# arnold117/PrimeKG-RGCN-LinkPrediction

Hardware: NVIDIA B200
Metric: rgcn_fwd_bwd_edges_per_sec (higher is better)
Workload: dtype bf16x3-split / f32-accumulate (operands as bf16 hi + lo planes, three tensor-core products, ~17 mantissa bits; gathers, means, loss in f32)

## Files before the change

primekg-rgcn-linkprediction_b200/csrc/aggregate.cu:

```cuda
#include <stdlib.h>

#include <type_traits>

#include "common.cuh"

namespace rgcn {

enum { MIX_NONE = 0, MIX_SUM = 1, MIX_BASIS = 2 };
#ifndef RGCN_TAILPRED_MAX_VPL
#define RGCN_TAILPRED_MAX_VPL 1
#endif
constexpr int kMaxBasis = 8;

struct AggParams {
  const int32_t* rowptr;
  const int32_t* idx;
  const float* edge_w;
  const int32_t* hub_keys;
  const int32_t* hub_chunk_ptr;
  const int32_t* chunk_table;
  const int32_t* row_order;
  int32_t hub_threshold;
  int32_t skip_hubs;
  int32_t n_hubs;
// ... 20 lines not shown
  int32_t out_mode;
  float* partials;
  const float* dotP;
  int64_t ld_dotP;
  float* gc_partial;
  const int32_t* slot;
  int32_t zero_row;
  const float* mp_mask; int64_t ld_mp_mask; float mp_scale;
  void* mp_hi; void* mp_lo; int64_t ld_mp;
  float* mp_colsum;
  const int64_t* list;
  int64_t n_list;
  int32_t list_slices, list_rsplit;
  int64_t list_walkers;
  int32_t list_by_rows;
  int32_t list_overlap_hubs;
  int32_t stream_rel;
  const uint8_t* row_flag;
  const int32_t* hub_filter;
  int32_t hub_unlisted;
};

template <int G, int VPL, bool W, bool SLOT = false>
__global__ void __launch_bounds__(256) hub_partial_kernel(const AggParams p) {
  pdl_enter();
  constexpr int GROUPS = 256 / G;
  __shared__ float4 red[GROUPS][G * VPL];
  const int chunk = blockIdx.x;
  const int4 t = __ldg(reinterpret_cast<const int4*>(p.chunk_table) + chunk);
  const int key = t.x;
  const int r = key % p.R;
  if (p.hub_filter && __ldg(p.hub_filter + key / p.R) == p.hub_unlisted) return;
  const int seg_beg = __ldg(p.rowptr + key), seg_end = __ldg(p.rowptr + key + 1);
  const int c_beg = seg_beg + (chunk - t.y) * kHubChunk;
  const int c_end = min(c_beg + kHubChunk, seg_end);
  const int nvec = p.d >> 2;
  const int lane = threadIdx.x % G, grp = threadIdx.x / G;
  constexpr int PER = kHubChunk / GROUPS;
  const int g_beg = c_beg + grp * PER, g_end = min(g_beg + PER, c_end);
  float4 acc[VPL];
  int vcol[VPL];
#pragma unroll
  for (int k = 0; k < VPL; ++k) {
    acc[k] = make_float4(0.f, 0.f, 0.f, 0.f);
    const int vi = k * G + lane;
    vcol[k] = vi < nvec ? vi * 4 : 0;
  }
  const float* __restrict__ Fb = p.F + (size_t)r * p.src_rel_stride;
// ... 43 lines not shown
    const float* __restrict__ rp = Fb + (size_t)j * ldf;
#pragma unroll
    for (int k = 0; k < VPL; ++k) {
      const float4 v = ldg4(rp + vcol[k]);
      if (W) fma4(acc[k], wv, v); else add4(acc[k], v);
    }
  }
#pragma unroll
  for (int k = 0; k < VPL; ++k) red[grp][k * G + lane] = acc[k];
  __syncthreads();
  for (int vi = threadIdx.x; vi < nvec; vi += 256) {
    float4 s = red[0][vi];
    for (int g = 1; g < GROUPS; ++g) add4(s, red[g][vi]);
    reinterpret_cast<float4*>(p.partials + (size_t)chunk * p.d)[vi] = s;
  }
}

__device__ __forceinline__ void store_vec_to(void* O, void* O_lo, int64_t ldo, int out_mode, int64_t row, int col,
                                             const float4& v) {
  if (out_mode == 0) {
    *reinterpret_cast<float4*>(reinterpret_cast<float*>(O) + row * ldo + col) = v;
    return;
  }
  __nv_bfloat162 a = __floats2bfloat162_rn(v.x, v.y), b = __floats2bfloat162_rn(v.z, v.w);
  uint2 hi;
  hi.x = *reinterpret_cast<uint32_t*>(&a);
  hi.y = *reinterpret_cast<uint32_t*>(&b);
  *reinterpret_cast<uint2*>(reinterpret_cast<__nv_bfloat16*>(O) + row * ldo + col) = hi;
  if (out_mode == 2) {
    const float hx = __uint_as_float(hi.x << 16), hy = __uint_as_float(hi.x & 0xffff0000u);
    const float hz = __uint_as_float(hi.y << 16), hw = __uint_as_float(hi.y & 0xffff0000u);
    a = __floats2bfloat162_rn(v.x - hx, v.y - hy);
    b = __floats2bfloat162_rn(v.z - hz, v.w - hw);
    uint2 lo;
    lo.x = *reinterpret_cast<uint32_t*>(&a);
    lo.y = *reinterpret_cast<uint32_t*>(&b);
    *reinterpret_cast<uint2*>(reinterpret_cast<__nv_bfloat16*>(O_lo) + row * ldo + col) = lo;
  }
}
__device__ __forceinline__ void store_vec(const AggParams& p, int64_t row, int col, const float4& v) {
  store_vec_to(p.O, p.O_lo, p.ldo, p.out_mode, row, col, v);
}

constexpr int agg_min_blocks(int G, int vpl, int mix, bool w) {
  if (mix == MIX_BASIS || vpl > 2) return 1;
  if (vpl == 2) return (mix == MIX_NONE && !w) ? 5 : 4;
  if (G == 32) return mix == MIX_NONE ? 6 : 5;
  return (mix == MIX_SUM && w) ? 3 : 4;
}

template <int G, int VPL, int MIX, bool W, bool SLOT = false, bool MP = false, bool LIST = false, bool MARK = false>
__global__ void __launch_bounds__(256, LIST ? (VPL > 2 ? 1 : 3) : agg_min_blocks(G, VPL, MIX, W) - (((MP || MARK) && agg_min_blocks(G, VPL, MIX, W) > 1) ? 1 : 0))
aggregate_rows_kernel(const AggParams p) {
  static_assert(!MARK || (SLOT && !MP && MIX == MIX_SUM), "marked sources serve the row-sparse backward walk");
  static_assert(!LIST || (MIX == MIX_NONE && !W && !SLOT && !MP), "the listed-rows walk is the unmixed forward form");
  pdl_enter();
  constexpr int GROUPS = 256 / G;
  constexpr int NB = (MIX == MIX_BASIS) ? kMaxBasis : 1;
  constexpr int U0 = (VPL >= 4) ? 2 : (VPL == 2 ? 4 : 8);
  constexpr int U = U0 < G ? U0 : G;
  constexpr bool TAILPRED = MIX != MIX_BASIS && VPL <= RGCN_TAILPRED_MAX_VPL;
  constexpr bool CHAIN = MIX == MIX_SUM && W;
  extern __shared__ float s_comp[];
  const bool with_gc = MIX == MIX_BASIS && p.dotP != nullptr;
  const bool with_cs = MP && MIX == MIX_SUM && p.mp_colsum != nullptr;
  float* s_gc = s_comp + p.R * p.B;
  if (MIX == MIX_BASIS) {
    for (int t = threadIdx.x; t < p.R * p.B; t += 256) s_comp[t] = p.comp[(t / p.B) * p.ldcomp + (t % p.B)];
    if (with_gc)
      for (int t = threadIdx.x; t < GROUPS * p.R * p.B; t += 256) s_gc[t] = 0.f;
    __syncthreads();
// ... 142 lines not shown
        while (e + U <= cend) fbatch(std::integral_constant<int, U>{}, false);
        const int n_left = cend - e;
        if (n_left == 1) fbatch(std::integral_constant<int, 1>{}, false);
        else if (n_left == 2) fbatch(std::integral_constant<int, (U >= 2 ? 2 : 1)>{}, U < 2);
        else if (n_left > 0 && n_left <= 4 && U > 4) fbatch(std::integral_constant<int, (U > 4 ? 4 : 1)>{}, true);
        else if (n_left > 0) fbatch(std::integral_constant<int, U>{}, true);
        continue;
      }
    }
    for (int rr = 0; rr < rcount; ++rr) {
      const int r = rbase + rr;
      const int beg = __shfl_sync(gmask, my_beg, rr, G);
      const int end = __shfl_sync(gmask, my_end, rr, G);
      const int len = end - beg;
      if (len == 0 && MIX != MIX_NONE) continue;
      if (MIX != MIX_BASIS && p.skip_hubs && len > p.hub_threshold) continue;
      float4 acc[VPL];
      const bool chained = CHAIN && len <= p.hub_threshold;
#pragma unroll
      for (int k = 0; k < VPL; ++k) acc[k] = chained ? mix[0][k] : make_float4(0.f, 0.f, 0.f, 0.f);
      if (len > p.hub_threshold) {
        const int key = (int)(key0 + r);
        int lo = 0, hi = p.n_hubs;
        while (hi - lo > 1) {
          int mid = (lo + hi) >> 1;
          if (__ldg(p.hub_keys + mid) <= key) lo = mid; else hi = mid;
        }
        const int c0 = __ldg(p.hub_chunk_ptr + lo), c1 = __ldg(p.hub_chunk_ptr + lo + 1);
        int c = c0;
        for (; c + U <= c1; c += U) {
          float4 v[U][VPL];
// ... 272 lines not shown
    }
  }
  if (MIX == MIX_SUM) {
    float* o = reinterpret_cast<float*>(p.O) + row * p.ldo;
#pragma unroll
    for (int k = 0; k < VPL; ++k) {
      if (act[k]) {
        float4 cur = *reinterpret_cast<const float4*>(o + vcol[k]);
        add4(cur, total[k]);
        *reinterpret_cast<float4*>(o + vcol[k]) = cur;
      }
    }
  }
}

template <int G, int VPL>
__global__ void __launch_bounds__(256) hub_finish_list_kernel(const AggParams p) {
  pdl_enter();
  constexpr int GROUPS = 256 / G;
  const int lane = threadIdx.x % G;
  const int h = blockIdx.x * GROUPS + threadIdx.x / G;
  if (h >= p.n_hubs) return;
  const int key = __ldg(p.hub_keys + h);
  const int64_t row = key / p.R;
  const int r = key - (int)row * p.R;
  const int64_t orow = __ldg(p.hub_filter + row);
  if (orow == p.hub_unlisted) return;
  const int d = p.d, nvec = p.d >> 2;
  const int c0 = __ldg(p.hub_chunk_ptr + h), c1 = __ldg(p.hub_chunk_ptr + h + 1);
  const float len = (float)(__ldg(p.rowptr + key + 1) - __ldg(p.rowptr + key));
  constexpr int U = (VPL >= 4) ? 2 : (VPL == 2 ? 4 : 8);
#pragma unroll
  for (int k = 0; k < VPL; ++k) {
    const int vi = k * G + lane;
    if (vi >= nvec) continue;
    float4 acc = make_float4(0.f, 0.f, 0.f, 0.f);
    int c = c0;
    for (; c + U <= c1; c += U) {
      float4 v[U];
#pragma unroll
      for (int u = 0; u < U; ++u) v[u] = *reinterpret_cast<const float4*>(p.partials + (size_t)(c + u) * d + vi * 4);
#pragma unroll
      for (int u = 0; u < U; ++u) add4(acc, v[u]);
    }
    for (; c < c1; ++c) add4(acc, *reinterpret_cast<const float4*>(p.partials + (size_t)c * d + vi * 4));
    acc = div4(acc, len);
    store_vec(p, orow, r * p.block_stride + vi * 4, acc);
  }
}

struct f8 { float v[8]; };
__device__ __forceinline__ void ld_bf8(const __nv_bfloat16* p, uint4& raw) { raw = __ldg(reinterpret_cast<const uint4*>(p)); }
__device__ __forceinline__ void acc_bf8(f8& a, const uint4& r) {
  const uint32_t w[4] = {r.x, r.y, r.z, r.w};
#pragma unroll
  for (int i = 0; i < 4; ++i) {
    unsigned long long acc2 = pack2(a.v[2 * i], a.v[2 * i + 1]);
    const unsigned long long x2 = pack2(__uint_as_float(w[i] << 16), __uint_as_float(w[i] & 0xffff0000u));
    asm("add.rn.f32x2 %0, %0, %1;" : "+l"(acc2) : "l"(x2));
    unpack2(acc2, a.v[2 * i], a.v[2 * i + 1]);
  }
}
__device__ __forceinline__ uint4 pack_bf8(const f8& a) {
  uint4 o;
  __nv_bfloat162 t;
// ... 229 lines not shown
  cudaStream_t side = nullptr;
  cudaEvent_t fork = nullptr, join = nullptr;
};
static ForkJoin* fork_join() {
  static ForkJoin fj[64];
  int dev = 0;
  if (cudaGetDevice(&dev) != cudaSuccess || dev < 0 || dev >= 64) return nullptr;
  ForkJoin& f = fj[dev];
  if (!f.side) {
    if (cudaStreamCreateWithFlags(&f.side, cudaStreamNonBlocking) != cudaSuccess) return nullptr;
    if (cudaEventCreateWithFlags(&f.fork, cudaEventDisableTiming) != cudaSuccess) return nullptr;
    if (cudaEventCreateWithFlags(&f.join, cudaEventDisableTiming) != cudaSuccess) return nullptr;
  }
  return &f;
}
static ForkJoin* fork_join_existing(cudaStream_t st) {
  static ForkJoin* made[64] = {nullptr};
  int dev = 0;
  if (cudaGetDevice(&dev) != cudaSuccess || dev < 0 || dev >= 64) return nullptr;
  if (made[dev]) return made[dev];
  cudaStreamCaptureStatus cs = cudaStreamCaptureStatusNone;
  if (cudaStreamIsCapturing(st, &cs) != cudaSuccess || cs != cudaStreamCaptureStatusNone) return nullptr;
  made[dev] = fork_join();
  return made[dev];
}
static bool overlap_hubs_enabled() {
  const char* e = getenv("RGCN_OVERLAP_HUBS");
  return e && e[0] == '1';
}

template <int G, int VPL, int MIX, bool W>
static int launch_agg_overlapped(AggParams p, int n_chunks, cudaStream_t st) {
  if (!p.range_mode) { p.row_begin = 0; p.row_end = p.n_rows; }
  constexpr int GROUPS = 256 / G;
  ForkJoin* fj = fork_join();
  if (!fj) { set_error("aggregate: could not create the side stream for the hub pass"); return RGCN_ECUDA; }
  p.skip_hubs = 1;
  RGCN_CUDA(cudaEventRecord(fj->fork, st));
  RGCN_CUDA(cudaStreamWaitEvent(fj->side, fj->fork, 0));
  hub_partial_kernel<G, VPL, W><<<n_chunks, 256, 0, fj->side>>>(p);
  RGCN_LAUNCH_CHECK();
  RGCN_CUDA(cudaEventRecord(fj->join, fj->side));
  const unsigned grid = (unsigned)((p.n_rows + GROUPS - 1) / GROUPS);
// ... 8 lines not shown
template <int G, int VPL>
static int launch_agg(const AggParams& p_in, int mix, int n_chunks, cudaStream_t st) {
  constexpr int GROUPS = 256 / G;
  AggParams p = p_in;
  if (!p.range_mode) { p.row_begin = 0; p.row_end = p.n_rows; }
  if (p.no_hub_pass) n_chunks = 0;
  const int64_t n_walk = p.row_end - p.row_begin;
  if (!p.list && !p.slot && !p.mp_hi && n_chunks > 0 && p.n_rows > 0 && n_walk == p.n_rows && mix != MIX_BASIS && overlap_hubs_enabled() && (mix == MIX_NONE || p.out_mode == 0)) {
    const bool w = p.edge_w != nullptr;
    if (mix == MIX_NONE)
      return w ? launch_agg_overlapped<G, VPL, MIX_NONE, true>(p, n_chunks, st) : launch_agg_overlapped<G, VPL, MIX_NONE, false>(p, n_chunks, st);
    return w ? launch_agg_overlapped<G, VPL, MIX_SUM, true>(p, n_chunks, st) : launch_agg_overlapped<G, VPL, MIX_SUM, false>(p, n_chunks, st);
  }
  if (p.list) {
    if (mix != MIX_NONE || p.edge_w || p.slot || p.mp_hi) { set_error("aggregate: the listed-rows walk serves the unmixed forward only"); return RGCN_EINVAL; }
    const dim3 lgrid((unsigned)((n_walk + GROUPS - 1) / GROUPS), (unsigned)(p.list_slices > 0 ? p.list_slices : 1),
                     (unsigned)(p.list_rsplit > 0 ? p.list_rsplit : 1));
    ForkJoin* fj = (p.list_overlap_hubs && n_chunks > 0 && n_walk > 0 && p.list_slices <= 1) ? fork_join_existing(st) : nullptr;
    if (fj) {
      RGCN_CUDA(cudaEventRecord(fj->fork, st));
      RGCN_CUDA(cudaStreamWaitEvent(fj->side, fj->fork, 0));
      hub_partial_kernel<G, VPL, false><<<n_chunks, 256, 0, fj->side>>>(p);
      RGCN_LAUNCH_CHECK();
      RGCN_CUDA(cudaEventRecord(fj->join, fj->side));
      p.skip_hubs = 1;
      RGCN_CUDA(launch_pdl(aggregate_rows_kernel<G, VPL, MIX_NONE, false, false, false, true>, lgrid, dim3(256), 0, st, p));
      RGCN_LAUNCH_CHECK();
      RGCN_CUDA(cudaStreamWaitEvent(st, fj->join, 0));
      hub_finish_list_kernel<G, VPL><<<(unsigned)((p.n_hubs + GROUPS - 1) / GROUPS), 256, 0, st>>>(p);
      RGCN_LAUNCH_CHECK();
      return RGCN_OK;
    }
    if (n_chunks > 0) {
      RGCN_CUDA(launch_pdl(hub_partial_kernel<G, VPL, false>, dim3(n_chunks), dim3(256), 0, st, p));
      RGCN_LAUNCH_CHECK();
    }
    if (n_walk <= 0) return RGCN_OK;
    RGCN_CUDA(launch_pdl(aggregate_rows_kernel<G, VPL, MIX_NONE, false, false, false, true>, lgrid, dim3(256), 0, st, p));
    RGCN_LAUNCH_CHECK();
    return RGCN_OK;
  }
  if (p.slot) {
    if (mix != MIX_SUM || !p.edge_w) { set_error("aggregate: the row-sparse gather serves the backward walk only"); return RGCN_EINVAL; }
    if (n_chunks > 0) {
      RGCN_CUDA(launch_pdl(hub_partial_kernel<G, VPL, true, true>, dim3(n_chunks), dim3(256), 0, st, p));
      RGCN_LAUNCH_CHECK();
    }
    if (n_walk <= 0) return RGCN_OK;
    const dim3 sgrid((unsigned)((n_walk + GROUPS - 1) / GROUPS));
    if (p.mp_hi) RGCN_CUDA(launch_pdl(aggregate_rows_kernel<G, VPL, MIX_SUM, true, true, true>, sgrid, dim3(256),
                                      p.mp_colsum ? (size_t)GROUPS * p.d * sizeof(float) : 0, st, p));
    else if (p.row_flag) RGCN_CUDA(launch_pdl(aggregate_rows_kernel<G, VPL, MIX_SUM, true, true, false, false, true>, sgrid, dim3(256), 0, st, p));
    else RGCN_CUDA(launch_pdl(aggregate_rows_kernel<G, VPL, MIX_SUM, true, true>, sgrid, dim3(256), 0, st, p));
    RGCN_LAUNCH_CHECK();
    return RGCN_OK;
  }
  if (n_chunks > 0) {
    if (p.edge_w) RGCN_CUDA(launch_pdl(hub_partial_kernel<G, VPL, true>, dim3(n_chunks), dim3(256), 0, st, p));
    else RGCN_CUDA(launch_pdl(hub_partial_kernel<G, VPL, false>, dim3(n_chunks), dim3(256), 0, st, p));
    RGCN_LAUNCH_CHECK();
  }
  if (n_walk <= 0) return RGCN_OK;
  const unsigned grid = (unsigned)((n_walk + GROUPS - 1) / GROUPS);
  const bool w = p.edge_w != nullptr;
  const size_t sm = (size_t)p.R * p.B * sizeof(float) * (p.dotP ? 1 + GROUPS : 1);
  if (mix == MIX_NONE) {
    if (w) RGCN_CUDA(launch_pdl(aggregate_rows_kernel<G, VPL, MIX_NONE, true>, dim3(grid), dim3(256), 0, st, p));
    else RGCN_CUDA(launch_pdl(aggregate_rows_kernel<G, VPL, MIX_NONE, false>, dim3(grid), dim3(256), 0, st, p));
// ... 25 lines not shown

static int check_common(const rgcn_csr_t* g, const float* F, int64_t ldf, int32_t d, const void* ws,
                        size_t ws_bytes) {
  RGCN_CHECK_ARG(g && g->rowptr && (g->idx || g->E == 0), "aggregate: null CSR arrays");
  RGCN_CHECK_ARG(g->R >= 1 && g->n_rows >= 0, "aggregate: bad n_rows/R");
  RGCN_CHECK_ARG(g->hub_threshold >= 1, "aggregate: hub_threshold must be the (positive) threshold the hub plan was made with");
  RGCN_CHECK_ARG(d >= 4 && d <= 1024 && d % 4 == 0, "aggregate: feature width d=%d must be a multiple of 4 in [4,1024]", d);
  RGCN_CHECK_ARG(F && ldf % 4 == 0 && ((uintptr_t)F & 15) == 0, "aggregate: feature matrix must be 16-byte aligned with ld %% 4 == 0");
  RGCN_CHECK_ARG(g->n_chunks == 0 || (g->hub_keys && g->hub_chunk_ptr && g->n_hubs > 0 && g->chunk_table &&
                                      ((uintptr_t)g->chunk_table & 15) == 0), "aggregate: hub plan missing");
  if (g->n_chunks > 0 && (!ws || ws_bytes < (size_t)g->n_chunks * d * sizeof(float))) {
    set_error("aggregate: workspace too small (%zu < %zu)", ws_bytes, (size_t)g->n_chunks * d * sizeof(float));
    return RGCN_EWORKSPACE;
  }
  return RGCN_OK;
}

}

using namespace rgcn;

extern "C" size_t rgcn_aggregate_workspace_bytes(const rgcn_csr_t* g, int32_t d) {
  if (!g) return 0;
  return align_up((size_t)g->n_chunks * (size_t)d * sizeof(float), 256);
}

constexpr int kBasisSlice = 128;

static int64_t agg_blocks(int64_t n_rows, int d) {
  const int nvec = d >> 2;
// ... 21 lines not shown
  RGCN_CHECK_ARG(!dot_p || (comp && B <= kMaxBasis && gc_partial && ((uintptr_t)dot_p & 15) == 0 && ld_dot_p % 4 == 0),
                 "aggregate_fwd: the coefficient-gradient side output needs comp, B <= %d, aligned P and a partial buffer", kMaxBasis);
  RGCN_CHECK_ARG(out_mode >= 0 && out_mode <= 2, "aggregate_fwd: out_mode must be 0 (fp32), 1 (bf16) or 2 (bf16 hi+lo)");
  RGCN_CHECK_ARG(H && ((uintptr_t)H & (out_mode ? 7 : 15)) == 0 && ldh % 4 == 0, "aggregate_fwd: output must be aligned with ld %% 4 == 0");
  RGCN_CHECK_ARG(out_mode != 2 || (H_lo && ((uintptr_t)H_lo & 7) == 0), "aggregate_fwd: out_mode 2 needs the lo plane");
  RGCN_CHECK_ARG(!comp || (B >= 1), "aggregate_fwd: bad number of bases");
  AggParams p{};
  p.rowptr = g->rowptr; p.idx = g->idx; p.edge_w = g->w;
  p.hub_keys = g->hub_keys; p.hub_chunk_ptr = g->hub_chunk_ptr; p.n_hubs = g->n_hubs; p.chunk_table = g->chunk_table;
  p.row_order = g->row_order; p.hub_threshold = g->hub_threshold;
  p.n_rows = g->n_rows; p.R = g->R;
  p.F = X; p.ldf = ldx; p.src_rel_stride = 0; p.d = d; p.block_stride = d;
  p.O = H; p.O_lo = H_lo; p.ldo = ldh; p.out_mode = out_mode; p.partials = (float*)workspace;
  p.dotP = dot_p; p.ld_dotP = ld_dot_p; p.gc_partial = gc_partial;
  p.root_rows = x_root; p.ld_root = ld_x_root;
  cudaStream_t st = (cudaStream_t)stream;
  if (!comp) return dispatch_agg(p, MIX_NONE, g->n_chunks, st);
  int64_t gc_row = 0;
  const int slice = dot_p ? kBasisSlice : d;
  for (int b0 = 0; b0 < B; b0 += kMaxBasis) {
    for (int c0 = 0; c0 < d; c0 += slice) {
      const int dc = d - c0 < slice ? d - c0 : slice;
      AggParams q = p;
      q.comp = comp + b0; q.ldcomp = B; q.B = (B - b0 < kMaxBasis) ? (B - b0) : kMaxBasis;
      q.F = X + c0; q.d = dc;
      const size_t off = (size_t)b0 * d + c0;
      q.O = out_mode ? (void*)((__nv_bfloat16*)H + off) : (void*)((float*)H + off);
      if (out_mode == 2) q.O_lo = (void*)((__nv_bfloat16*)H_lo + off);
      q.partials = (float*)workspace + (size_t)g->n_chunks * c0;
      if (dot_p) {
// ... 19 lines not shown
  RGCN_CHECK_ARG(H && ((uintptr_t)H & (out_mode ? 7 : 15)) == 0 && ldh % 4 == 0, "aggregate_fwd_rows: output must be aligned with ld %% 4 == 0");
  RGCN_CHECK_ARG(out_mode != 2 || (H_lo && ((uintptr_t)H_lo & 7) == 0), "aggregate_fwd_rows: out_mode 2 needs the lo plane");
  RGCN_CHECK_ARG(0 <= row_begin && row_begin <= row_end && row_end <= g->n_rows, "aggregate_fwd_rows: bad row range");
  RGCN_CHECK_ARG(!g->row_order || g->order_chunk_rows == 0 ||
                 ((row_begin % g->order_chunk_rows == 0) && (row_end % g->order_chunk_rows == 0 || row_end == g->n_rows)),
                 "aggregate_fwd_rows: with a chunk-wise row order the range must consist of whole order chunks");
  RGCN_CHECK_ARG(!g->row_order || g->order_chunk_rows > 0 || (row_begin == 0 && row_end == g->n_rows) || row_begin == row_end,
                 "aggregate_fwd_rows: a global row order cannot be walked in ranges");
  AggParams p{};
  p.rowptr = g->rowptr; p.idx = g->idx; p.edge_w = g->w;
  p.hub_keys = g->hub_keys; p.hub_chunk_ptr = g->hub_chunk_ptr; p.n_hubs = g->n_hubs; p.chunk_table = g->chunk_table;
  p.row_order = g->row_order; p.hub_threshold = g->hub_threshold;
  p.n_rows = g->n_rows; p.R = g->R;
  p.F = X; p.ldf = ldx; p.src_rel_stride = 0; p.d = d; p.block_stride = d;
  p.O = H; p.O_lo = H_lo; p.ldo = ldh; p.out_mode = out_mode; p.partials = (float*)workspace;
  p.root_rows = x_root; p.ld_root = ld_x_root;
  p.range_mode = 1; p.row_begin = row_begin; p.row_end = row_end; p.no_hub_pass = hub_pass ? 0 : 1;
  if (row_end == row_begin && !hub_pass) return RGCN_OK;
  return dispatch_agg(p, MIX_NONE, g->n_chunks, (cudaStream_t)stream);
}

extern "C" int rgcn_aggregate_fwd_bf16(const rgcn_csr_t* g, const void* X16, int64_t ldx, int32_t d, void* H_hi, int64_t ldh,
                                       const void* x_root16, int64_t ld_x_root, int64_t row_begin, int64_t row_end,
                                       int32_t hub_pass, void* workspace, size_t workspace_bytes, rgcn_stream_t stream) {
  RGCN_CHECK_ARG(g && g->rowptr && (g->idx || g->E == 0) && g->R >= 1 && g->n_rows >= 0 && g->hub_threshold >= 1, "aggregate_fwd_bf16: bad CSR");
  RGCN_CHECK_ARG(d >= 8 && d <= 1024 && d % 8 == 0, "aggregate_fwd_bf16: d=%d must be a multiple of 8 in [8, 1024]", d);
  RGCN_CHECK_ARG(X16 && ((uintptr_t)X16 & 15) == 0 && ldx % 8 == 0, "aggregate_fwd_bf16: features must be 16-byte aligned rows");
  RGCN_CHECK_ARG(H_hi && ((uintptr_t)H_hi & 15) == 0 && ldh % 8 == 0, "aggregate_fwd_bf16: output plane must be 16-byte aligned, ld %% 8 == 0");
  RGCN_CHECK_ARG(!x_root16 || (((uintptr_t)x_root16 & 15) == 0 && ld_x_root % 8 == 0), "aggregate_fwd_bf16: x_root misaligned");
  RGCN_CHECK_ARG(0 <= row_begin && row_begin <= row_end && row_end <= g->n_rows, "aggregate_fwd_bf16: bad row range");
  RGCN_CHECK_ARG(g->n_chunks == 0 || (g->hub_keys && g->hub_chunk_ptr && g->n_hubs > 0 && g->chunk_table), "aggregate_fwd_bf16: hub plan missing");
// ... 120 lines not shown
  RGCN_CHECK_ARG(rows && slot && n_list > 0 && n_list < (1ll << 30), "aggregate_fwd_list: bad row list / slot map");
  const int64_t m_c = rgcn_rows_compact_size(n_list);
  RGCN_CHECK_ARG(g->n_chunks == 0 || (g->hub_keys && g->hub_chunk_ptr && g->n_hubs > 0 && g->chunk_table), "aggregate_fwd_list: hub plan missing");
  if (g->n_chunks > 0 && (!workspace || workspace_bytes < (size_t)g->n_chunks * d * sizeof(float))) {
    set_error("aggregate_fwd_list: workspace too small"); return RGCN_EWORKSPACE;
  }
  AggParams p{};
  p.rowptr = g->rowptr; p.idx = g->idx;
  p.hub_keys = g->hub_keys; p.hub_chunk_ptr = g->hub_chunk_ptr; p.n_hubs = g->n_hubs; p.chunk_table = g->chunk_table;
  p.hub_threshold = g->hub_threshold;
  p.n_rows = g->n_rows; p.R = g->R;
  p.F = (const float*)X; p.ldf = ldx; p.src_rel_stride = 0; p.d = d; p.block_stride = d;
  p.O = H; p.O_lo = H_lo; p.ldo = ldh; p.out_mode = out_mode; p.partials = (float*)workspace;
  p.root_rows = (const float*)x_root; p.ld_root = ld_x_root;
  p.list = rows; p.n_list = n_list; p.hub_filter = slot; p.hub_unlisted = (int32_t)m_c;
  static int env_by_rows = -1;
  if (env_by_rows < 0) { const char* e = getenv("RGCN_LIST_BY_ROWS"); env_by_rows = e ? atoi(e) : 0; }
  p.list_by_rows = env_by_rows == 2 ? (g->n_rows <= 16 * n_list ? 1 : 0) : (env_by_rows ? 1 : 0);
  p.row_order = p.list_by_rows ? g->row_order : nullptr;
  p.list_walkers = p.list_by_rows ? g->n_rows : n_list;
  p.range_mode = 1; p.row_begin = 0; p.row_end = p.list_walkers + m_c;
  cudaStream_t st = (cudaStream_t)stream;
  auto run = [&](const AggParams& q, int n_chunks) {
    if (!x_bf16) return dispatch_agg(q, MIX_NONE, n_chunks, st);
    const int nvec = q.d >> 3;
    if (nvec <= 4) return launch_agg_bf16<4, 1>(q, n_chunks, st);
    if (nvec <= 8) return launch_agg_bf16<8, 1>(q, n_chunks, st);
    if (nvec <= 16) return launch_agg_bf16<16, 1>(q, n_chunks, st);
    if (nvec <= 32) return launch_agg_bf16<32, 1>(q, n_chunks, st);
    if (nvec <= 64) return launch_agg_bf16<32, 2>(q, n_chunks, st);
    return launch_agg_bf16<32, 4>(q, n_chunks, st);
  };
  static int env_overlap = -1;
  if (env_overlap < 0) { const char* e = getenv("RGCN_LIST_OVERLAP_HUBS"); env_overlap = e ? atoi(e) : 0; }
  static int env_slice0 = -1;
  if (env_slice0 < 0) { const char* e = getenv("RGCN_LIST_SLICE"); env_slice0 = e ? atoi(e) : 0; }
  if (!x_bf16 && env_overlap && env_slice0 == 0 && g->n_chunks > 0) {
    cudaStreamCaptureStatus cs = cudaStreamCaptureStatusNone;
    const bool capturing = cudaStreamIsCapturing(st, &cs) == cudaSuccess && cs == cudaStreamCaptureStatusActive;
    if (!capturing) (void)fork_join_existing(st);
    if (env_overlap == 1 || capturing) {
      static int env_rs = -1;
      if (env_rs < 0) { const char* e = getenv("RGCN_LIST_RSPLIT"); env_rs = e ? atoi(e) : 1; }
      p.list_overlap_hubs = 1; p.list_slices = 1;
      p.list_rsplit = env_rs < 1 ? 1 : (env_rs > g->R ? g->R : env_rs);
      return run(p, g->n_chunks);
    }
  }
  if (g->n_chunks > 0) {
    AggParams h = p;
    h.row_end = h.row_begin;
    int rc = run(h, g->n_chunks);
    if (rc) return rc;
  }
  static int env_slice = -1, env_rsplit = -1;
  if (env_slice < 0) { const char* e = getenv("RGCN_LIST_SLICE"); env_slice = e ? atoi(e) : 0; }
  if (env_rsplit < 0) { const char* e = getenv("RGCN_LIST_RSPLIT"); env_rsplit = e ? atoi(e) : 1; }
  const int unit = x_bf16 ? 8 : 4;
  int slice = d;
  if (env_slice >= unit && env_slice % unit == 0 && env_slice < d && d % env_slice == 0) slice = env_slice;
  p.d = slice; p.list_slices = d / slice;
  p.list_rsplit = env_rsplit < 1 ? 1 : (env_rsplit > g->R ? g->R : env_rsplit);
  p.no_hub_pass = 1;
  return run(p, 0);
}

extern "C" int rgcn_aggregate_fwd_list(const rgcn_csr_t* g, const float* X, int64_t ldx, int32_t d, void* H, void* H_lo,
                                       int64_t ldh, int32_t out_mode, const float* x_root, int64_t ld_x_root,
                                       const int64_t* rows, int64_t n_list, const int32_t* slot, void* workspace,
                                       size_t workspace_bytes, rgcn_stream_t stream) {
  RGCN_CHECK_ARG(d >= 4 && d <= 1024 && d % 4 == 0, "aggregate_fwd_list: feature width d=%d must be a multiple of 4 in [4,1024]", d);
  RGCN_CHECK_ARG(X && ldx % 4 == 0 && ((uintptr_t)X & 15) == 0, "aggregate_fwd_list: feature matrix must be 16-byte aligned with ld %% 4 == 0");
  RGCN_CHECK_ARG(!x_root || (((uintptr_t)x_root & 15) == 0 && ld_x_root % 4 == 0), "aggregate_fwd_list: x_root misaligned");
  RGCN_CHECK_ARG(out_mode >= 0 && out_mode <= 2, "aggregate_fwd_list: out_mode must be 0 (fp32), 1 (bf16) or 2 (bf16 hi+lo)");
  RGCN_CHECK_ARG(H && ((uintptr_t)H & (out_mode ? 7 : 15)) == 0 && ldh % 4 == 0, "aggregate_fwd_list: output must be aligned with ld %% 4 == 0");
  RGCN_CHECK_ARG(out_mode != 2 || (H_lo && ((uintptr_t)H_lo & 7) == 0), "aggregate_fwd_list: out_mode 2 needs the lo plane");
  return aggregate_fwd_list_impl(g, X, ldx, d, false, H, H_lo, ldh, out_mode, x_root, ld_x_root, rows, n_list, slot, workspace,
// ... 14 lines not shown
```

primekg-rgcn-linkprediction_b200/csrc/csr_build.cu:

```cuda
#include <cub/cub.cuh>

#include "common.cuh"

namespace rgcn {

__global__ void make_keys_kernel(const int64_t* __restrict__ major, const int64_t* __restrict__ minor,
                                 const int64_t* __restrict__ rel, int64_t E, int64_t n_major, int64_t n_minor,
                                 int32_t R, int major_bit, int minor_bit,
                                 uint32_t* __restrict__ keys, int32_t* __restrict__ vals,
                                 int32_t* __restrict__ hist, int32_t* __restrict__ status) {
  const int64_t stride = (int64_t)gridDim.x * blockDim.x;
  for (int64_t e = (int64_t)blockIdx.x * blockDim.x + threadIdx.x; e < E; e += stride) {
    const int64_t a = major[e], b = minor[e], r = rel[e];
    int bad = 0;
    if (a < 0 || a >= n_major) bad |= major_bit;
    if (b < 0 || b >= n_minor) bad |= minor_bit;
    if (r < 0 || r >= R) bad |= 4;
    uint32_t k = 0;
    if (bad) {
      atomicOr(status, bad);
    } else {
      k = (uint32_t)(a * R + r);
      atomicAdd(hist + k, 1);
    }
// ... 111 lines not shown
    c = (rowptr[k + 1] - rowptr[k] + kHubChunk - 1) / kHubChunk;
  }
  chunk_cnt[h] = c;
}

__global__ void hub_chunk_table_kernel(const int32_t* __restrict__ hub_keys, const int32_t* __restrict__ chunk_ptr,
                                       int n_hubs, int R, int4* __restrict__ table) {
  const int h = blockIdx.x * blockDim.x + threadIdx.x;
  if (h >= n_hubs) return;
  const int key = hub_keys[h], row = key / R;
  int first = h, end = h + 1;
  while (first > 0 && hub_keys[first - 1] / R == row) --first;
  while (end < n_hubs && hub_keys[end] / R == row) ++end;
  const int need = chunk_ptr[end] - chunk_ptr[first];
  const int c0 = chunk_ptr[h], c1 = chunk_ptr[h + 1];
  for (int c = c0; c < c1; ++c) table[c] = make_int4(key, c0, first, need);
}

}

using namespace rgcn;

extern "C" int rgcn_hub_chunk_table(const int32_t* hub_keys, const int32_t* hub_chunk_ptr, int32_t n_hubs, int32_t R,
                                    int32_t* chunk_table, rgcn_stream_t stream) {
  RGCN_CHECK_ARG(n_hubs >= 0 && R >= 1, "hub_chunk_table: bad sizes");
  if (n_hubs == 0) return RGCN_OK;
  RGCN_CHECK_ARG(hub_keys && hub_chunk_ptr && chunk_table && ((uintptr_t)chunk_table & 15) == 0,
                 "hub_chunk_table: null or misaligned argument");
  hub_chunk_table_kernel<<<(unsigned)((n_hubs + 127) / 128), 128, 0, (cudaStream_t)stream>>>(
      hub_keys, hub_chunk_ptr, n_hubs, R, reinterpret_cast<int4*>(chunk_table));
  RGCN_LAUNCH_CHECK();
// ... 91 lines not shown
```

primekg-rgcn-linkprediction_b200/graph.py:

```python
from __future__ import annotations

import ctypes as C
import os
import weakref
from collections import OrderedDict
from typing import Optional

import torch

from . import _lib


def _ptr(t: Optional[torch.Tensor]):
    return None if t is None else C.c_void_p(t.data_ptr())


_raw_stream = getattr(torch._C, "_cuda_getCurrentRawStream", None)


def _stream_id(device) -> int:
    if _raw_stream is not None:
        idx = device.index if isinstance(device, torch.device) else torch.device(device).index
        if idx is None:
            idx = torch.cuda.current_device()
# ... 50 lines not shown
        lib = _lib.load()
        dev = self.rowptr.device
        cap = self.E // self.threshold + 1
        n_keys = self.n_rows * self.R
        hub_keys = torch.empty(cap, dtype=torch.int32, device=dev)
        chunk_ptr = torch.empty(cap + 1, dtype=torch.int32, device=dev)
        ws_bytes = lib.rgcn_hub_plan_workspace_bytes(n_keys, cap)
        ws = torch.empty(ws_bytes, dtype=torch.uint8, device=dev)
        nh, nc = C.c_int32(0), C.c_int32(0)
        _lib.check(lib.rgcn_hub_plan(_ptr(self.rowptr), n_keys, self.threshold, _ptr(hub_keys), _ptr(chunk_ptr), cap,
                                     C.byref(nh), C.byref(nc), _ptr(ws), ws_bytes, _stream(dev)), "rgcn_hub_plan")
        self.n_hubs, self.n_chunks = int(nh.value), int(nc.value)
        if self.n_hubs:
            self.hub_keys = hub_keys[: self.n_hubs].clone()
            self.hub_chunk_ptr = chunk_ptr[: self.n_hubs + 1].clone()
            self.chunk_table = torch.empty(self.n_chunks, 4, dtype=torch.int32, device=dev)
            _lib.check(lib.rgcn_hub_chunk_table(_ptr(self.hub_keys), _ptr(self.hub_chunk_ptr), self.n_hubs, self.R,
                                                _ptr(self.chunk_table), _stream(dev)), "rgcn_hub_chunk_table")

    def workspace(self, d: int) -> Optional[torch.Tensor]:
        if self.n_chunks == 0:
            return None
        ws = self._ws.get(d)
        if ws is None:
            ws = torch.empty(self.n_chunks * d + 64, dtype=torch.float32, device=self.rowptr.device)
            self._ws[d] = ws
        return ws


class RelGraph:

# ... 105 lines not shown
```

Measured before the change: 2.858 billion.

## Fuse hub partial and finish passes into the aggregate kernel via last-block counters

Appends hub-chunk blocks to the unmixed forward aggregate grid. Each hub block writes its partial sum, then bumps an atomic per-hub counter stored after the chunk table, and the last block to finish reduces all partials and writes the mean. This removes the separate hub-partial and hub-finish launches and the side-stream fork/join. The cost is threadfences, atomics and a serial tail reduction in one block per hub. It is gated to walks of at most 65536 rows and can be disabled with an environment variable.

Result: faster. 2.926 billion (median of 6 runs) (+2.4%).

```diff
diff --git a/primekg-rgcn-linkprediction_b200/csrc/aggregate.cu b/primekg-rgcn-linkprediction_b200/csrc/aggregate.cu
--- a/primekg-rgcn-linkprediction_b200/csrc/aggregate.cu
+++ b/primekg-rgcn-linkprediction_b200/csrc/aggregate.cu
@@ -58,24 +58,24 @@
   int32_t list_slices, list_rsplit;
   int64_t list_walkers;
   int32_t list_by_rows;
-  int32_t list_overlap_hubs;
+  int32_t hub_block0;
+  int32_t* hub_cnt;
   int32_t stream_rel;
   const uint8_t* row_flag;
   const int32_t* hub_filter;
   int32_t hub_unlisted;
 };
 
-template <int G, int VPL, bool W, bool SLOT = false>
-__global__ void __launch_bounds__(256) hub_partial_kernel(const AggParams p) {
-  pdl_enter();
+template <int G, int VPL, bool W, bool SLOT>
+__device__ __forceinline__ bool hub_chunk_partial(const AggParams& p, int chunk, int4& t, int& len) {
   constexpr int GROUPS = 256 / G;
   __shared__ float4 red[GROUPS][G * VPL];
-  const int chunk = blockIdx.x;
-  const int4 t = __ldg(reinterpret_cast<const int4*>(p.chunk_table) + chunk);
+  t = __ldg(reinterpret_cast<const int4*>(p.chunk_table) + chunk);
   const int key = t.x;
   const int r = key % p.R;
-  if (p.hub_filter && __ldg(p.hub_filter + key / p.R) == p.hub_unlisted) return;
+  if (p.hub_filter && __ldg(p.hub_filter + key / p.R) == p.hub_unlisted) return false;
   const int seg_beg = __ldg(p.rowptr + key), seg_end = __ldg(p.rowptr + key + 1);
+  len = seg_end - seg_beg;
   const int c_beg = seg_beg + (chunk - t.y) * kHubChunk;
   const int c_end = min(c_beg + kHubChunk, seg_end);
   const int nvec = p.d >> 2;
@@ -149,6 +149,15 @@
     for (int g = 1; g < GROUPS; ++g) add4(s, red[g][vi]);
     reinterpret_cast<float4*>(p.partials + (size_t)chunk * p.d)[vi] = s;
   }
+  return true;
+}
+
+template <int G, int VPL, bool W, bool SLOT = false>
+__global__ void __launch_bounds__(256) hub_partial_kernel(const AggParams p) {
+  pdl_enter();
+  int4 t;
+  int len;
+  (void)hub_chunk_partial<G, VPL, W, SLOT>(p, blockIdx.x, t, len);
 }
 
 __device__ __forceinline__ void store_vec_to(void* O, void* O_lo, int64_t ldo, int out_mode, int64_t row, int col,
@@ -177,6 +186,56 @@
   store_vec_to(p.O, p.O_lo, p.ldo, p.out_mode, row, col, v);
 }
 
+template <int G, int VPL, bool LIST>
+__device__ __forceinline__ void hub_chunk_role(const AggParams& p, int chunk) {
+  __shared__ int s_last;
+  int4 t;
+  int len;
+  if (!hub_chunk_partial<G, VPL, false, false>(p, chunk, t, len)) return;
+  const int c0 = t.y, nch = (len + kHubChunk - 1) / kHubChunk;
+  __threadfence();
+  __syncthreads();
+  if (threadIdx.x == 0) s_last = atomicAdd(p.hub_cnt + c0, 1) == nch - 1;
+  __syncthreads();
+  if (!s_last) return;
+  __threadfence();
+  const int key = t.x;
+  const int64_t row = key / p.R;
+  const int r = key - (int)row * p.R;
+  const int64_t orow = LIST ? (int64_t)__ldg(p.hub_filter + row) : row;
+  const int d = p.d, nvec = p.d >> 2;
+  constexpr int NV = G * VPL;
+  constexpr int S = NV >= 256 ? 1 : (256 / NV >= 32 ? 32 : 256 / NV);
+  constexpr int L = S >= 16 ? 1 : 16 / S;
+  const int slot = threadIdx.x % S;
+  const unsigned smask = (S == 32) ? 0xffffffffu : (((1u << S) - 1u) << ((threadIdx.x & 31) / S * S));
+  for (int vi = threadIdx.x / S; vi < nvec; vi += 256 / S) {
+    const float* __restrict__ src = p.partials + (size_t)c0 * d + vi * 4;
+    float4 acc = make_float4(0.f, 0.f, 0.f, 0.f);
+    for (int c = 0; c < nch; c += S * L) {
+      float4 v[L];
+#pragma unroll
+      for (int u = 0; u < L; ++u) {
+        const int cu = c + slot * L + u;
+        v[u] = cu < nch ? __ldcg(reinterpret_cast<const float4*>(src + (size_t)cu * d)) : make_float4(0.f, 0.f, 0.f, 0.f);
+      }
+      for (int s = 0; s < S; ++s) {
+#pragma unroll
+        for (int u = 0; u < L; ++u) {
+          float4 w = v[u];
+          if (S > 1) {
+            w.x = __shfl_sync(smask, w.x, s, S); w.y = __shfl_sync(smask, w.y, s, S);
+            w.z = __shfl_sync(smask, w.z, s, S); w.w = __shfl_sync(smask, w.w, s, S);
+          }
+          if (c + s * L + u < nch) add4(acc, w);
+        }
+      }
+    }
+    if (slot == 0) store_vec(p, orow, r * p.block_stride + vi * 4, div4(acc, (float)len));
+  }
+  if (threadIdx.x == 0) p.hub_cnt[c0] = 0;
+}
+
 constexpr int agg_min_blocks(int G, int vpl, int mix, bool w) {
   if (mix == MIX_BASIS || vpl > 2) return 1;
   if (vpl == 2) return (mix == MIX_NONE && !w) ? 5 : 4;
@@ -184,12 +243,17 @@
   return (mix == MIX_SUM && w) ? 3 : 4;
 }
 
-template <int G, int VPL, int MIX, bool W, bool SLOT = false, bool MP = false, bool LIST = false, bool MARK = false>
+template <int G, int VPL, int MIX, bool W, bool SLOT = false, bool MP = false, bool LIST = false, bool MARK = false, bool HUBS = false>
 __global__ void __launch_bounds__(256, LIST ? (VPL > 2 ? 1 : 3) : agg_min_blocks(G, VPL, MIX, W) - (((MP || MARK) && agg_min_blocks(G, VPL, MIX, W) > 1) ? 1 : 0))
 aggregate_rows_kernel(const AggParams p) {
   static_assert(!MARK || (SLOT && !MP && MIX == MIX_SUM), "marked sources serve the row-sparse backward walk");
   static_assert(!LIST || (MIX == MIX_NONE && !W && !SLOT && !MP), "the listed-rows walk is the unmixed forward form");
+  static_assert(!HUBS || (MIX == MIX_NONE && !W && !SLOT && !MP && !MARK), "hub segments finish themselves in the unmixed forward walk");
   pdl_enter();
+  if (HUBS && blockIdx.x >= (unsigned)p.hub_block0) {
+    hub_chunk_role<G, VPL, LIST>(p, (int)(blockIdx.x - p.hub_block0));
+    return;
+  }
   constexpr int GROUPS = 256 / G;
   constexpr int NB = (MIX == MIX_BASIS) ? kMaxBasis : 1;
   constexpr int U0 = (VPL >= 4) ? 2 : (VPL == 2 ? 4 : 8);
@@ -362,7 +426,7 @@
       const int end = __shfl_sync(gmask, my_end, rr, G);
       const int len = end - beg;
       if (len == 0 && MIX != MIX_NONE) continue;
-      if (MIX != MIX_BASIS && p.skip_hubs && len > p.hub_threshold) continue;
+      if (MIX != MIX_BASIS && (HUBS || p.skip_hubs) && len > p.hub_threshold) continue;
       float4 acc[VPL];
       const bool chained = CHAIN && len <= p.hub_threshold;
 #pragma unroll
@@ -665,41 +729,6 @@
   }
 }
 
-template <int G, int VPL>
-__global__ void __launch_bounds__(256) hub_finish_list_kernel(const AggParams p) {
-  pdl_enter();
-  constexpr int GROUPS = 256 / G;
-  const int lane = threadIdx.x % G;
-  const int h = blockIdx.x * GROUPS + threadIdx.x / G;
-  if (h >= p.n_hubs) return;
-  const int key = __ldg(p.hub_keys + h);
-  const int64_t row = key / p.R;
-  const int r = key - (int)row * p.R;
-  const int64_t orow = __ldg(p.hub_filter + row);
-  if (orow == p.hub_unlisted) return;
-  const int d = p.d, nvec = p.d >> 2;
-  const int c0 = __ldg(p.hub_chunk_ptr + h), c1 = __ldg(p.hub_chunk_ptr + h + 1);
-  const float len = (float)(__ldg(p.rowptr + key + 1) - __ldg(p.rowptr + key));
-  constexpr int U = (VPL >= 4) ? 2 : (VPL == 2 ? 4 : 8);
-#pragma unroll
-  for (int k = 0; k < VPL; ++k) {
-    const int vi = k * G + lane;
-    if (vi >= nvec) continue;
-    float4 acc = make_float4(0.f, 0.f, 0.f, 0.f);
-    int c = c0;
-    for (; c + U <= c1; c += U) {
-      float4 v[U];
-#pragma unroll
-      for (int u = 0; u < U; ++u) v[u] = *reinterpret_cast<const float4*>(p.partials + (size_t)(c + u) * d + vi * 4);
-#pragma unroll
-      for (int u = 0; u < U; ++u) add4(acc, v[u]);
-    }
-    for (; c < c1; ++c) add4(acc, *reinterpret_cast<const float4*>(p.partials + (size_t)c * d + vi * 4));
-    acc = div4(acc, len);
-    store_vec(p, orow, r * p.block_stride + vi * 4, acc);
-  }
-}
-
 struct f8 { float v[8]; };
 __device__ __forceinline__ void ld_bf8(const __nv_bfloat16* p, uint4& raw) { raw = __ldg(reinterpret_cast<const uint4*>(p)); }
 __device__ __forceinline__ void acc_bf8(f8& a, const uint4& r) {
@@ -959,19 +988,16 @@
   }
   return &f;
 }
-static ForkJoin* fork_join_existing(cudaStream_t st) {
-  static ForkJoin* made[64] = {nullptr};
-  int dev = 0;
-  if (cudaGetDevice(&dev) != cudaSuccess || dev < 0 || dev >= 64) return nullptr;
-  if (made[dev]) return made[dev];
-  cudaStreamCaptureStatus cs = cudaStreamCaptureStatusNone;
-  if (cudaStreamIsCapturing(st, &cs) != cudaSuccess || cs != cudaStreamCaptureStatusNone) return nullptr;
-  made[dev] = fork_join();
-  return made[dev];
-}
 static bool overlap_hubs_enabled() {
   const char* e = getenv("RGCN_OVERLAP_HUBS");
   return e && e[0] == '1';
+}
+
+constexpr int64_t kSelfFinishMaxRows = 65536;
+static bool hubs_self_finish(const AggParams& p, int n_chunks, int64_t n_walk) {
+  if (n_chunks <= 0 || n_walk <= 0 || n_walk > kSelfFinishMaxRows || !p.hub_cnt) return false;
+  const char* e = getenv("RGCN_HUB_SELF_FINISH");
+  return !(e && e[0] == '0');
 }
 
 template <int G, int VPL, int MIX, bool W>
@@ -1010,23 +1036,15 @@
   }
   if (p.list) {
     if (mix != MIX_NONE || p.edge_w || p.slot || p.mp_hi) { set_error("aggregate: the listed-rows walk serves the unmixed forward only"); return RGCN_EINVAL; }
-    const dim3 lgrid((unsigned)((n_walk + GROUPS - 1) / GROUPS), (unsigned)(p.list_slices > 0 ? p.list_slices : 1),
-                     (unsigned)(p.list_rsplit > 0 ? p.list_rsplit : 1));
-    ForkJoin* fj = (p.list_overlap_hubs && n_chunks > 0 && n_walk > 0 && p.list_slices <= 1) ? fork_join_existing(st) : nullptr;
-    if (fj) {
-      RGCN_CUDA(cudaEventRecord(fj->fork, st));
-      RGCN_CUDA(cudaStreamWaitEvent(fj->side, fj->fork, 0));
-      hub_partial_kernel<G, VPL, false><<<n_chunks, 256, 0, fj->side>>>(p);
-      RGCN_LAUNCH_CHECK();
-      RGCN_CUDA(cudaEventRecord(fj->join, fj->side));
-      p.skip_hubs = 1;
-      RGCN_CUDA(launch_pdl(aggregate_rows_kernel<G, VPL, MIX_NONE, false, false, false, true>, lgrid, dim3(256), 0, st, p));
-      RGCN_LAUNCH_CHECK();
-      RGCN_CUDA(cudaStreamWaitEvent(st, fj->join, 0));
-      hub_finish_list_kernel<G, VPL><<<(unsigned)((p.n_hubs + GROUPS - 1) / GROUPS), 256, 0, st>>>(p);
+    const unsigned wblocks = (unsigned)((n_walk + GROUPS - 1) / GROUPS);
+    if (hubs_self_finish(p, n_chunks, n_walk) && p.list_slices <= 1 && p.list_rsplit <= 1) {
+      p.hub_block0 = (int32_t)wblocks;
+      RGCN_CUDA(launch_pdl(aggregate_rows_kernel<G, VPL, MIX_NONE, false, false, false, true, false, true>,
+                           dim3((unsigned)n_chunks + wblocks), dim3(256), 0, st, p));
       RGCN_LAUNCH_CHECK();
       return RGCN_OK;
     }
+    const dim3 lgrid(wblocks, (unsigned)(p.list_slices > 0 ? p.list_slices : 1), (unsigned)(p.list_rsplit > 0 ? p.list_rsplit : 1));
     if (n_chunks > 0) {
       RGCN_CUDA(launch_pdl(hub_partial_kernel<G, VPL, false>, dim3(n_chunks), dim3(256), 0, st, p));
       RGCN_LAUNCH_CHECK();
@@ -1048,6 +1066,14 @@
                                       p.mp_colsum ? (size_t)GROUPS * p.d * sizeof(float) : 0, st, p));
     else if (p.row_flag) RGCN_CUDA(launch_pdl(aggregate_rows_kernel<G, VPL, MIX_SUM, true, true, false, false, true>, sgrid, dim3(256), 0, st, p));
     else RGCN_CUDA(launch_pdl(aggregate_rows_kernel<G, VPL, MIX_SUM, true, true>, sgrid, dim3(256), 0, st, p));
+    RGCN_LAUNCH_CHECK();
+    return RGCN_OK;
+  }
+  if (mix == MIX_NONE && !p.edge_w && hubs_self_finish(p, n_chunks, n_walk)) {
+    const unsigned wblocks = (unsigned)((n_walk + GROUPS - 1) / GROUPS);
+    p.hub_block0 = (int32_t)wblocks;
+    RGCN_CUDA(launch_pdl(aggregate_rows_kernel<G, VPL, MIX_NONE, false, false, false, false, false, true>,
+                         dim3((unsigned)n_chunks + wblocks), dim3(256), 0, st, p));
     RGCN_LAUNCH_CHECK();
     return RGCN_OK;
   }
@@ -1103,6 +1129,10 @@
     return RGCN_EWORKSPACE;
   }
   return RGCN_OK;
+}
+
+static int32_t* hub_counters(const rgcn_csr_t* g) {
+  return g->n_chunks > 0 ? const_cast<int32_t*>(g->chunk_table) + 4 * (size_t)g->n_chunks : nullptr;
 }
 
 }
@@ -1154,6 +1184,7 @@
   p.O = H; p.O_lo = H_lo; p.ldo = ldh; p.out_mode = out_mode; p.partials = (float*)workspace;
   p.dotP = dot_p; p.ld_dotP = ld_dot_p; p.gc_partial = gc_partial;
   p.root_rows = x_root; p.ld_root = ld_x_root;
+  p.hub_cnt = hub_counters(g);
   cudaStream_t st = (cudaStream_t)stream;
   if (!comp) return dispatch_agg(p, MIX_NONE, g->n_chunks, st);
   int64_t gc_row = 0;
@@ -1203,7 +1234,7 @@
   p.n_rows = g->n_rows; p.R = g->R;
   p.F = X; p.ldf = ldx; p.src_rel_stride = 0; p.d = d; p.block_stride = d;
   p.O = H; p.O_lo = H_lo; p.ldo = ldh; p.out_mode = out_mode; p.partials = (float*)workspace;
-  p.root_rows = x_root; p.ld_root = ld_x_root;
+  p.root_rows = x_root; p.ld_root = ld_x_root; p.hub_cnt = hub_counters(g);
   p.range_mode = 1; p.row_begin = row_begin; p.row_end = row_end; p.no_hub_pass = hub_pass ? 0 : 1;
   if (row_end == row_begin && !hub_pass) return RGCN_OK;
   return dispatch_agg(p, MIX_NONE, g->n_chunks, (cudaStream_t)stream);
@@ -1354,6 +1385,7 @@
   p.O = H; p.O_lo = H_lo; p.ldo = ldh; p.out_mode = out_mode; p.partials = (float*)workspace;
   p.root_rows = (const float*)x_root; p.ld_root = ld_x_root;
   p.list = rows; p.n_list = n_list; p.hub_filter = slot; p.hub_unlisted = (int32_t)m_c;
+  if (!x_bf16) p.hub_cnt = hub_counters(g);
   static int env_by_rows = -1;
   if (env_by_rows < 0) { const char* e = getenv("RGCN_LIST_BY_ROWS"); env_by_rows = e ? atoi(e) : 0; }
   p.list_by_rows = env_by_rows == 2 ? (g->n_rows <= 16 * n_list ? 1 : 0) : (env_by_rows ? 1 : 0);
@@ -1371,36 +1403,25 @@
     if (nvec <= 64) return launch_agg_bf16<32, 2>(q, n_chunks, st);
     return launch_agg_bf16<32, 4>(q, n_chunks, st);
   };
-  static int env_overlap = -1;
-  if (env_overlap < 0) { const char* e = getenv("RGCN_LIST_OVERLAP_HUBS"); env_overlap = e ? atoi(e) : 0; }
-  static int env_slice0 = -1;
-  if (env_slice0 < 0) { const char* e = getenv("RGCN_LIST_SLICE"); env_slice0 = e ? atoi(e) : 0; }
-  if (!x_bf16 && env_overlap && env_slice0 == 0 && g->n_chunks > 0) {
-    cudaStreamCaptureStatus cs = cudaStreamCaptureStatusNone;
-    const bool capturing = cudaStreamIsCapturing(st, &cs) == cudaSuccess && cs == cudaStreamCaptureStatusActive;
-    if (!capturing) (void)fork_join_existing(st);
-    if (env_overlap == 1 || capturing) {
-      static int env_rs = -1;
-      if (env_rs < 0) { const char* e = getenv("RGCN_LIST_RSPLIT"); env_rs = e ? atoi(e) : 1; }
-      p.list_overlap_hubs = 1; p.list_slices = 1;
-      p.list_rsplit = env_rs < 1 ? 1 : (env_rs > g->R ? g->R : env_rs);
-      return run(p, g->n_chunks);
-    }
-  }
-  if (g->n_chunks > 0) {
-    AggParams h = p;
-    h.row_end = h.row_begin;
-    int rc = run(h, g->n_chunks);
-    if (rc) return rc;
-  }
   static int env_slice = -1, env_rsplit = -1;
   if (env_slice < 0) { const char* e = getenv("RGCN_LIST_SLICE"); env_slice = e ? atoi(e) : 0; }
   if (env_rsplit < 0) { const char* e = getenv("RGCN_LIST_RSPLIT"); env_rsplit = e ? atoi(e) : 1; }
   const int unit = x_bf16 ? 8 : 4;
   int slice = d;
   if (env_slice >= unit && env_slice % unit == 0 && env_slice < d && d % env_slice == 0) slice = env_slice;
+  const int rsplit = env_rsplit < 1 ? 1 : (env_rsplit > g->R ? g->R : env_rsplit);
+  if (slice == d && rsplit == 1 && hubs_self_finish(p, g->n_chunks, p.row_end - p.row_begin)) {
+    p.list_slices = 1; p.list_rsplit = 1;
+    return run(p, g->n_chunks);
+  }
+  if (g->n_chunks > 0) {
+    AggParams h = p;
+    h.row_end = h.row_begin;
+    int rc = run(h, g->n_chunks);
+    if (rc) return rc;
+  }
   p.d = slice; p.list_slices = d / slice;
-  p.list_rsplit = env_rsplit < 1 ? 1 : (env_rsplit > g->R ? g->R : env_rsplit);
+  p.list_rsplit = rsplit;
   p.no_hub_pass = 1;
   return run(p, 0);
 }
diff --git a/primekg-rgcn-linkprediction_b200/csrc/csr_build.cu b/primekg-rgcn-linkprediction_b200/csrc/csr_build.cu
--- a/primekg-rgcn-linkprediction_b200/csrc/csr_build.cu
+++ b/primekg-rgcn-linkprediction_b200/csrc/csr_build.cu
@@ -149,7 +149,11 @@
   while (end < n_hubs && hub_keys[end] / R == row) ++end;
   const int need = chunk_ptr[end] - chunk_ptr[first];
   const int c0 = chunk_ptr[h], c1 = chunk_ptr[h + 1];
-  for (int c = c0; c < c1; ++c) table[c] = make_int4(key, c0, first, need);
+  int32_t* cnt = reinterpret_cast<int32_t*>(table + chunk_ptr[n_hubs]);
+  for (int c = c0; c < c1; ++c) {
+    table[c] = make_int4(key, c0, first, need);
+    cnt[c] = 0;
+  }
 }
 
 }
diff --git a/primekg-rgcn-linkprediction_b200/graph.py b/primekg-rgcn-linkprediction_b200/graph.py
--- a/primekg-rgcn-linkprediction_b200/graph.py
+++ b/primekg-rgcn-linkprediction_b200/graph.py
@@ -88,7 +88,7 @@
         if self.n_hubs:
             self.hub_keys = hub_keys[: self.n_hubs].clone()
             self.hub_chunk_ptr = chunk_ptr[: self.n_hubs + 1].clone()
-            self.chunk_table = torch.empty(self.n_chunks, 4, dtype=torch.int32, device=dev)
+            self.chunk_table = torch.empty(self.n_chunks * 5, dtype=torch.int32, device=dev)
             _lib.check(lib.rgcn_hub_chunk_table(_ptr(self.hub_keys), _ptr(self.hub_chunk_ptr), self.n_hubs, self.R,
                                                 _ptr(self.chunk_table), _stream(dev)), "rgcn_hub_chunk_table")
 
```
